# mrafidashti/neuradar

Hardware: NVIDIA B200
Metric: train_step_rays_per_sec (higher is better)
Workload: dtype f32

## Files before the change

neuradar_b200/csrc/field_fused.cu:

```cuda
#include <algorithm>
#include <cstdlib>

#include <cuda.h>
#include <cuda_bf16.h>

#include "actor_grid.cuh"
#include "hash_bwd_plan.cuh"
#include "tc_common.cuh"

namespace nrb {

using namespace tc;

struct FusedParams {
  const float* w[5];
  const float* b[5];
  const float* beta;
  float beta_min;
};

__device__ constexpr int kLK[5] = {32, 32, 48, 32, 32};
__device__ constexpr int kLN[5] = {32, 48, 32, 32, 32};
__device__ constexpr int kLOut[5] = {32, 33, 32, 32, 32};

// ... 145 lines not shown
    int agid = -1;
    if constexpr (kActors) agid = __ldg(a.as.grid_id + rr);
    if (kActors && agid >= 0) {
      float o16[16];
      actor_gather16(a.ag, agid, __ldg(a.as.pos + 3 * rr), __ldg(a.as.pos + 3 * rr + 1), __ldg(a.as.pos + 3 * rr + 2),
                     __ldg(a.as.std + rr), o16);
#pragma unroll
      for (int j = 0; j < 16; ++j) {
        v[j] = o16[j];
        v[16 + j] = 0.0f;
      }
    } else if constexpr (F > 0) {
      const float px = __ldg(a.xyz + 3 * rr), py = __ldg(a.xyz + 3 * rr + 1), pz = __ldg(a.xyz + 3 * rr + 2);
      const float sd = a.std != nullptr ? __ldg(a.std + rr) : 0.0f;
      const uint32_t hmask = (1u << grid.log2_size) - 1u;
      constexpr int kBatch = 8 / F;
#pragma unroll
      for (int l0 = 0; l0 < 32 / F; l0 += kBatch) {
        Cell c[kBatch];
        float f[kBatch][8][F];
#pragma unroll
        for (int i = 0; i < kBatch; ++i) {
          c[i] = locate_cell(px, py, pz, grid.scalings[l0 + i], hmask);
          const float* base = grid.table + (static_cast<size_t>(l0 + i) << grid.log2_size) * F;
#pragma unroll
          for (int k = 0; k < 8; ++k) load_row<F>(base, c[i].row[k], f[i][k]);
        }
#pragma unroll
        for (int i = 0; i < kBatch; ++i) {
          const float ax = c[i].ox, bx = 1.0f - c[i].ox, ay = c[i].oy, by = 1.0f - c[i].oy, az = c[i].oz, bz = 1.0f - c[i].oz;
          const float w = a.std != nullptr ? level_weight(grid.scalings[l0 + i], sd) : 1.0f;
#pragma unroll
          for (int j = 0; j < F; ++j) {
            const float f03 = f[i][0][j] * ax + f[i][3][j] * bx;
            const float f12 = f[i][1][j] * ax + f[i][2][j] * bx;
            const float f56 = f[i][5][j] * ax + f[i][6][j] * bx;
            const float f47 = f[i][4][j] * ax + f[i][7][j] * bx;
            const float f0312 = f03 * ay + f12 * by;
            const float f4756 = f47 * ay + f56 * by;
            v[(l0 + i) * F + j] = (f0312 * az + f4756 * bz) * w;
          }
        }
      }
    } else {
      float4 pf[8];
      warp_load_rows_coalesced(a.x, tile * kRows + (uwarp & 3) * 32, a.M, lane, pf);
      warp_bounce_to_rows(bounce, lane, pf, v);
    }
    tmem_store_row_split<32>(tg, uwarp, kFAHi, kFALo, 0, v);
    if (train) {
#pragma unroll
      for (int q = 0; q < 4; ++q) {
        uint32_t h[4], m[4];
#pragma unroll
        for (int c = 0; c < 4; ++c) split_bf16_pair(v[8 * q + 2 * c], v[8 * q + 2 * c + 1], h[c], m[c]);
        uint4* dst = a.ximg + tile * 1024 + q * 128 + r;
        dst[0] = make_uint4(h[0], h[1], h[2], h[3]);
        dst[512] = make_uint4(m[0], m[1], m[2], m[3]);
      }
    }
    auto relu_mask = [&](const float* bias) {
      uint32_t m = 0;
#pragma unroll
      for (int j = 0; j < 32; ++j) {
        v[j] = fmaxf(v[j] + bias[j], 0.0f);
        m |= (v[j] > 0.0f ? 1u : 0u) << j;
      }
      return m;
    };
    run_layer(0);
    tmem_load_row<32>(tg + kFAcc, uwarp, 0, v);
    const uint32_t m_h1 = relu_mask(s_bias);
    tmem_store_row_split<32>(tg, uwarp, kFAHi, kFALo, 0, v);
    run_layer(1);
    float sdf_v;
    float emb[32];
    {
      float geo[48];
      tmem_load_row<48>(tg + kFAcc, uwarp, 0, geo);
      sdf_v = geo[0] + s_bias[48];
#pragma unroll
      for (int j = 0; j < 32; ++j) emb[j] = geo[1 + j] + s_bias[48 + 1 + j];
    }
    tmem_store_row_split<32>(tg, uwarp, kFAHi, kFALo, 0, emb);
    {
      float shv[16];
      if (kActors && agid >= 0) {
        sh16_of_direction(__ldg(a.as.dirs + 3 * rr), __ldg(a.as.dirs + 3 * rr + 1), __ldg(a.as.dirs + 3 * rr + 2), shv);
      } else {
        const float4* shp = reinterpret_cast<const float4*>(a.sh + (rr / a.samples_per_ray) * 16);
#pragma unroll
        for (int c = 0; c < 4; ++c) {
          const float4 q4 = __ldg(shp + c);
          shv[4 * c] = q4.x;
          shv[4 * c + 1] = q4.y;
          shv[4 * c + 2] = q4.z;
          shv[4 * c + 3] = q4.w;
        }
      }
      tmem_store_row_split<16>(tg, uwarp, kFAHi, kFALo, 32, shv);
    }
    run_layer(2);
    tmem_load_row<32>(tg + kFAcc, uwarp, 0, v);
    const uint32_t m_g1 = relu_mask(s_bias + 2 * 48);
    tmem_store_row_split<32>(tg, uwarp, kFAHi, kFALo, 0, v);
    run_layer(3);
    tmem_load_row<32>(tg + kFAcc, uwarp, 0, v);
    const uint32_t m_g2 = relu_mask(s_bias + 3 * 48);
    tmem_store_row_split<32>(tg, uwarp, kFAHi, kFALo, 0, v);
    if (train && ok) {
      a.masks[row] = m_h1;
      a.masks[a.ld + row] = m_g1;
      a.masks[2 * a.ld + row] = m_g2;
    }
    run_layer(4);
    tmem_load_row<32>(tg + kFAcc, uwarp, 0, v);
#pragma unroll
    for (int j = 0; j < 32; ++j) v[j] = emb[j] + (v[j] + s_bias[4 * 48 + j]);
    warp_store_rows_coalesced(a.feature, tile * kRows + (uwarp & 3) * 32, a.M, bounce, lane, v);
    if (ok) {
      a.sdf[row] = sdf_v;
      a.alpha[row] = 1.0f / (1.0f + expf(sdf_v * beta));
    }
  }
  fence_before_sync();
  __syncthreads();
  if (uwarp == 0) tmem_free<512>(*tmem_slot);
}

constexpr int kBGroups = 2;
constexpr int kBWorkers = kBGroups * kRows;
constexpr int kBIssuers = 1;
constexpr int kBThreads = kBWorkers + kBIssuers * 32;
constexpr int kBCols = 112;
constexpr int kBAcc = 0, kBAHi = 32, kBAMid = 56, kBDHi = 80, kBDMid = 96;
__device__ constexpr int kDwCol[5] = {224, 224, 368, 296, 296};
__device__ constexpr int kDwLane[5] = {0, 16, 0, 0, 16};
constexpr int kSdfCol = 368, kSdfLane = 16;

struct FusedBwdSmem {
  static constexpr int d_hi = 0, d_mid = 8192;
  static constexpr int d_sdf = 16384;
  static constexpr int d_bytes = 18432;
  static constexpr int h1 = d_bytes;
  static constexpr int emb = h1 + 18432;
  static constexpr int g1 = emb + 26624;
  static constexpr int g2x = g1 + 18432;
  static constexpr int group_bytes = g2x + 18432;
  static constexpr int w = kBGroups * group_bytes;
  static constexpr int w_bytes = 4 * 4096 + 6144;
  static constexpr int w1row0 = w + w_bytes;
  static constexpr int bias = w1row0 + 128;
  static constexpr int mbar = bias + 5 * 48 * 4;
  static constexpr int tmem = mbar + 8 * 26;
  static constexpr int total = tmem + 16;
};
__host__ __device__ constexpr int fb_w_off(int l) { return l <= 2 ? l * 4096 : 4096 * 2 + 6144 + (l - 3) * 4096; }
__host__ __device__ constexpr int fb_w_half(int l) { return l == 2 ? 3072 : 2048; }
__device__ constexpr int kSlotOff[5] = {FusedBwdSmem::g2x, FusedBwdSmem::h1, FusedBwdSmem::emb, FusedBwdSmem::g1,
                                        FusedBwdSmem::g2x};
__device__ constexpr int kSlotMid[5] = {10240, 10240, 14336, 10240, 10240};

struct FusedBwdArgs {
  const uint4* ximg;
  const uint32_t* masks;
  int64_t ld;
  const float* sh;
  const float* sdf;
  const float* alpha;
  const float* dfeature;
  const float* dfeat_ray;
  const float* weights;
  const float* dsdf;
  const float* dalpha;
  int samples_per_ray;
  int64_t M;
  const int32_t* actor_grid_id;
  const float* actor_dirs;
  float4* dximg;
  float* dw[5];
  float* db[5];
  float* dbeta;
};

__device__ __forceinline__ void tmem_st16(uint32_t taddr, const uint32_t (&v)[16]) {
  asm volatile(
      "tcgen05.st.sync.aligned.32x32b.x16.b32 [%0], {%1, %2, %3, %4, %5, %6, %7, %8, %9, %10, %11, %12, %13, %14, %15, %16};" ::"r"(taddr),
      "r"(v[0]), "r"(v[1]), "r"(v[2]), "r"(v[3]), "r"(v[4]), "r"(v[5]), "r"(v[6]), "r"(v[7]), "r"(v[8]), "r"(v[9]), "r"(v[10]),
      "r"(v[11]), "r"(v[12]), "r"(v[13]), "r"(v[14]), "r"(v[15])
      : "memory");
}

__device__ __forceinline__ void tma_load_rows(void* dst_smem, const CUtensorMap* map, int32_t row0, uint64_t* mbar) {
  asm volatile(
      "cp.async.bulk.tensor.2d.shared::cluster.global.tile.mbarrier::complete_tx::bytes [%0], [%1, {%2, %3}], [%4];" ::"r"(
          smem_u32(dst_smem)),
      "l"(map), "r"(0), "r"(row0), "r"(smem_u32(mbar))
      : "memory");
}

#ifdef NRB_FUSED_TRACE
__device__ long long g_fused_trace[4096];
#define NRB_FT(slot)                                                                                            \
  do {                                                                                                          \
    if (blockIdx.x == 0 && t == 0 && trace_n < 2000) g_fused_trace[trace_n++] = (static_cast<long long>(slot) << 48) | (clock64() & 0xFFFFFFFFFFFFll); \
  } while (0)
#define NRB_FTI(slot)                                                                                           \
  do {                                                                                                          \
    if (blockIdx.x == 0 && uwarp == 8 && itrace_n < 4000) g_fused_trace[itrace_n++] = (static_cast<long long>(slot) << 48) | (clock64() & 0xFFFFFFFFFFFFll); \
  } while (0)
#else
#define NRB_FT(slot)
#define NRB_FTI(slot)
#endif

__global__ void __maxnreg__(128) field_fused_bwd_kernel(const __grid_constant__ FusedParams prm,
                                                                       const __grid_constant__ FusedBwdArgs a,
                                                                       const __grid_constant__ CUtensorMap dfeat_map) {
  extern __shared__ __align__(1024) char smem[];
  const int t = threadIdx.x, lane = t & 31, r = t & (kRows - 1);
  const int uwarp = uniform_warp_idx();
#ifdef NRB_FUSED_TRACE
  int trace_n = 0, itrace_n = 2000;
#endif
  uint64_t* mbars = reinterpret_cast<uint64_t*>(smem + FusedBwdSmem::mbar);
  uint64_t* mb_data = mbars;
  uint64_t* mb_xfull = mbars + 2;
  uint64_t* mb_dfull = mbars + 4;
  uint64_t* mb_ready = mbars + 6;
  uint64_t* mb_done = mbars + 16;
  uint32_t* tmem_slot = reinterpret_cast<uint32_t*>(smem + FusedBwdSmem::tmem);
  float* s_bias = reinterpret_cast<float*>(smem + FusedBwdSmem::bias);
  float* w1row0 = reinterpret_cast<float*>(smem + FusedBwdSmem::w1row0);

  for (int l = 0; l < 5; ++l) {
    const int K = kLK[l];
    const float* src = prm.w[l] + (l == 1 ? 32 : 0);
    char* hi = smem + FusedBwdSmem::w + fb_w_off(l);
    char* mid = hi + fb_w_half(l);
    for (int e = t; e < 32 * K / 2; e += kBThreads) {
      const int n = e / (K / 2), k = 2 * (e - n * (K / 2));
      uint32_t h, m;
      split_bf16_pair(__ldg(src + n * K + k), __ldg(src + n * K + k + 1), h, m);
      const int off = (n >> 3) * (K / 8) * 128 + (k >> 3) * 128 + (n & 7) * 16 + (k & 7) * 2;
      *reinterpret_cast<uint32_t*>(hi + off) = h;
      *reinterpret_cast<uint32_t*>(mid + off) = m;
    }
    for (int j = t; j < 48; j += kBThreads) s_bias[l * 48 + j] = (j < kLOut[l] && prm.b[l] != nullptr) ? __ldg(prm.b[l] + j) : 0.0f;
  }
  if (t < 32) w1row0[t] = __ldg(prm.w[1] + t);
  for (int gq = 0; gq < kBGroups; ++gq) {
    char* base = smem + gq * FusedBwdSmem::group_bytes;
    for (int e = t; e < 4 * 128; e += kBThreads) {
      const int slot = e >> 7, s = e & 127;
      const int off = slot == 0 ? FusedBwdSmem::h1 + 8192 : slot == 1 ? FusedBwdSmem::emb + 12288
                      : slot == 2 ? FusedBwdSmem::g1 + 8192 : FusedBwdSmem::g2x + 8192;
      *reinterpret_cast<uint4*>(base + off + s * 16) = make_uint4(0x00003F80u, 0u, 0u, 0u);
    }
  }
  if (uwarp == 0) tmem_alloc<512>(tmem_slot);
  if (t == 0) {
    for (int i = 0; i < 6; ++i) mbar_init(mbars + i, 1);
    for (int i = 0; i < 10; ++i) mbar_init(mb_ready + i, kRows);
    for (int i = 0; i < 10; ++i) mbar_init(mb_done + i, 1);
  }
  fence_async_smem();
  fence_before_sync();
  __syncthreads();
  fence_after_sync();
  const uint32_t tmem_base = *tmem_slot;
  const int64_t tiles = (a.M + kRows - 1) / kRows;
  const int64_t mine = static_cast<int64_t>(blockIdx.x) < tiles ? (tiles - 1 - blockIdx.x) / gridDim.x + 1 : 0;

  if (uwarp >= 8) {
    const int64_t cnt[2] = {(mine + 1) / 2, mine / 2};
    int64_t it[2] = {0, 0};
    int lcur[2] = {4, 4};
    bool pend[2] = {false, false};
    uint32_t used = 0;
    while (it[0] < cnt[0] || it[1] < cnt[1] || pend[0] || pend[1]) {
      bool progressed = false;
#pragma unroll
      for (int gq = 0; gq < 2; ++gq) {
        char* gsq = smem + gq * FusedBwdSmem::group_bytes;
        if (pend[gq] && mbar_test(mb_done + gq * 5 + 4, static_cast<uint32_t>(it[gq] & 1))) {
          if (elect_one()) {
            const int64_t tile = blockIdx.x + (2 * it[gq] + gq) * gridDim.x;
            mbar_expect_tx(mb_xfull + gq, 16384);
            bulk_load(gsq + FusedBwdSmem::g2x, a.ximg + tile * 1024, 8192, mb_xfull + gq);
            bulk_load(gsq + FusedBwdSmem::g2x + 10240, a.ximg + tile * 1024 + 512, 8192, mb_xfull + gq);
          }
          __syncwarp();
          pend[gq] = false;
          progressed = true;
        }
        if (it[gq] < cnt[gq] && mbar_test(mb_ready + gq * 5 + lcur[gq], static_cast<uint32_t>(it[gq] & 1))) {
          const int l = lcur[gq];
          if (elect_one()) {
            NRB_FTI(100 + gq);
            fence_after_sync();
            const uint32_t base = smem_u32(gsq);
            const uint32_t d_tmem = tmem_base + (static_cast<uint32_t>(kDwLane[l]) << 16) + static_cast<uint32_t>(kDwCol[l]);
            const uint32_t idesc = idesc_bf16(64, 2 * kLK[l] + 8, 1, 1);
            uint64_t da = make_desc(base + FusedBwdSmem::d_hi, 128, 2048), db = make_desc(base + kSlotOff[l], 128, 2048);
            const bool acc0 = (used >> l) & 1u;
#pragma unroll
            for (int ks = 0; ks < kRows / 16; ++ks) {
              mma_bf16_ss(d_tmem, da, db, idesc, acc0 || ks > 0);
              da += 16;
              db += 16;
            }
            if (l == 1) {
              const uint32_t s_tmem = tmem_base + (static_cast<uint32_t>(kSdfLane) << 16) + static_cast<uint32_t>(kSdfCol);
              uint64_t sa = make_desc(base + FusedBwdSmem::d_sdf, 128, 2048), sb = make_desc(base + kSlotOff[1], 128, 2048);
#pragma unroll
              for (int ks = 0; ks < kRows / 16; ++ks) {
                mma_bf16_ss(s_tmem, sa, sb, idesc, acc0 || ks > 0);
                sa += 16;
                sb += 16;
              }
            }
            mma_commit(mb_done + gq * 5 + l);
            NRB_FTI(110 + gq);
          }
          __syncwarp();
          used |= 1u << l;
          if (l == 4) pend[gq] = true;
          if (l == 0) {
            lcur[gq] = 4;
            ++it[gq];
          } else {
            lcur[gq] = l - 1;
          }
          progressed = true;
        }
      }
      if (!progressed) __nanosleep(64);
    }
  } else {
    const int g = uwarp >> 2, wq = uwarp & 3;
    char* gs = smem + g * FusedBwdSmem::group_bytes;
    const uint32_t tg = tmem_base + static_cast<uint32_t>(g * kBCols);
    const uint32_t lane_base = tg + (static_cast<uint32_t>(wq * 32) << 16);
    const float beta = fabsf(__ldg(prm.beta)) + prm.beta_min;
    const bool rank1 = a.dfeature == nullptr;
    uint32_t ph_data = 0;
    float dbeta_acc = 0.0f;

    auto data_step = [&](auto&& issue) {
      fence_before_sync();
      group_barrier(g);
      if (wq == 0) {
        if (elect_one()) {
          fence_after_sync();
          issue();
          mma_commit(mb_data + g);
        }
        __syncwarp();
      }
      mbar_wait(mb_data + g, ph_data);
      ph_data ^= 1;
      fence_after_sync();
    };
    auto issue_fwd = [&](int l) {
      const int K = kLK[l];
      const uint32_t idesc = idesc_bf16(128, 32, 0, 0);
      const uint32_t wb = smem_u32(smem + FusedBwdSmem::w + fb_w_off(l));
      uint64_t bh = make_desc(wb, 128, (K / 8) * 128), bm = make_desc(wb + fb_w_half(l), 128, (K / 8) * 128);
      for (int ks = 0; ks < K / 16; ++ks) {
        mma_bf16_ts(tg + kBAcc, tg + kBAMid + 8 * ks, bh, idesc, ks > 0);
        mma_bf16_ts(tg + kBAcc, tg + kBAHi + 8 * ks, bm, idesc, true);
        mma_bf16_ts(tg + kBAcc, tg + kBAHi + 8 * ks, bh, idesc, true);
        bh += 16;
        bm += 16;
      }
    };
    auto issue_din = [&](int l) {
      const int K = kLK[l];
      const uint32_t idesc = idesc_bf16(128, 32, 0, 1);
      const uint32_t wb = smem_u32(smem + FusedBwdSmem::w + fb_w_off(l));
      const uint32_t kgroup = static_cast<uint32_t>((K / 8) * 128);
      uint64_t bh = make_desc(wb, kgroup, 128), bm = make_desc(wb + fb_w_half(l), kgroup, 128);
      for (int ks = 0; ks < 2; ++ks) {
        mma_bf16_ts(tg + kBAcc, tg + kBDMid + 8 * ks, bh, idesc, ks > 0);
        mma_bf16_ts(tg + kBAcc, tg + kBDHi + 8 * ks, bm, idesc, true);
        mma_bf16_ts(tg + kBAcc, tg + kBDHi + 8 * ks, bh, idesc, true);
        bh += (2 * kgroup) >> 4;
        bm += (2 * kgroup) >> 4;
      }
    };
    auto stage_row32 = [&](const float (&v)[32], int col_hi, int col_mid, char* img_hi, char* img_mid) {
      uint32_t h[16], m[16];
#pragma unroll
      for (int c = 0; c < 16; ++c) split_bf16_pair(v[2 * c], v[2 * c + 1], h[c], m[c]);
      if (col_hi >= 0) {
        tmem_st16(lane_base + static_cast<uint32_t>(col_hi), h);
        tmem_st16(lane_base + static_cast<uint32_t>(col_mid), m);
      }
#pragma unroll
      for (int q = 0; q < 4; ++q) {
        *reinterpret_cast<uint4*>(img_hi + q * 2048 + r * 16) = make_uint4(h[4 * q], h[4 * q + 1], h[4 * q + 2], h[4 * q + 3]);
        *reinterpret_cast<uint4*>(img_mid + q * 2048 + r * 16) = make_uint4(m[4 * q], m[4 * q + 1], m[4 * q + 2], m[4 * q + 3]);
      }
      if (col_hi >= 0) tmem_st_wait();
    };
    auto load_acc = [&](float (&v)[32]) { tmem_load_row<32>(tg + kBAcc, uwarp, 0, v); };
    auto wait_done = [&](int l, int64_t it) { mbar_wait(mb_done + g * 5 + l, static_cast<uint32_t>(it & 1)); };
    auto signal_ready = [&](int l) {
      fence_async_smem();
      mbar_arrive(mb_ready + g * 5 + l);
    };

    uint4 xq[8];
    uint32_t m_h1 = 0, m_g1 = 0, m_g2 = 0;
    auto load_head = [&](int64_t tile) {
      const int64_t rc = min(tile * kRows + r, a.M - 1);
      const uint4* src = a.ximg + tile * 1024 + r;
#pragma unroll
      for (int q = 0; q < 4; ++q) {
        xq[q] = __ldg(src + q * 128);
        xq[4 + q] = __ldg(src + 512 + q * 128);
      }
      m_h1 = __ldg(a.masks + rc), m_g1 = __ldg(a.masks + a.ld + rc), m_g2 = __ldg(a.masks + 2 * a.ld + rc);
    };
    if (g < mine) load_head(blockIdx.x + static_cast<int64_t>(g) * gridDim.x);

    int64_t it = 0;
    for (int64_t k = g; k < mine; k += 2, ++it) {
      const int64_t tile = blockIdx.x + k * gridDim.x;
      const int64_t row = tile * kRows + r;
      const bool ok = row < a.M;
      const int64_t rc = ok ? row : (a.M - 1);
      float v[32];
      NRB_FT(0);
      if (it > 0) wait_done(0, it - 1);
      if (!rank1 && r == 0) {
        mbar_expect_tx(mb_dfull + g, 16384);
        tma_load_rows(gs + FusedBwdSmem::d_hi, &dfeat_map, static_cast<int32_t>(tile * kRows), mb_dfull + g);
      }
      {
        const uint32_t ha[16] = {xq[0].x, xq[0].y, xq[0].z, xq[0].w, xq[1].x, xq[1].y, xq[1].z, xq[1].w,
                                 xq[2].x, xq[2].y, xq[2].z, xq[2].w, xq[3].x, xq[3].y, xq[3].z, xq[3].w};
        const uint32_t ma[16] = {xq[4].x, xq[4].y, xq[4].z, xq[4].w, xq[5].x, xq[5].y, xq[5].z, xq[5].w,
                                 xq[6].x, xq[6].y, xq[6].z, xq[6].w, xq[7].x, xq[7].y, xq[7].z, xq[7].w};
        tmem_st16(lane_base + kBAHi, ha);
        tmem_st16(lane_base + kBAMid, ma);
        tmem_st_wait();
      }
      const uint32_t mh1 = m_h1, mg1 = m_g1, mg2 = m_g2;
      float4 shq[4];
      if (a.actor_grid_id != nullptr && __ldg(a.actor_grid_id + rc) >= 0) {
        float o[16];
        sh16_of_direction(__ldg(a.actor_dirs + 3 * rc), __ldg(a.actor_dirs + 3 * rc + 1), __ldg(a.actor_dirs + 3 * rc + 2), o);
#pragma unroll
        for (int c = 0; c < 4; ++c) shq[c] = make_float4(o[4 * c], o[4 * c + 1], o[4 * c + 2], o[4 * c + 3]);
      } else {
        const float4* shp = reinterpret_cast<const float4*>(a.sh + (rc / a.samples_per_ray) * 16);
#pragma unroll
        for (int c = 0; c < 4; ++c) shq[c] = __ldg(shp + c);
      }
      NRB_FT(10);
      data_step([&] { issue_fwd(0); });
      NRB_FT(20);
      load_acc(v);
#pragma unroll
      for (int j = 0; j < 32; ++j) v[j] = ((mh1 >> j) & 1u) ? v[j] + s_bias[j] : 0.0f;
      stage_row32(v, kBAHi, kBAMid, gs + FusedBwdSmem::h1, gs + FusedBwdSmem::h1 + 10240);
      NRB_FT(11);
      data_step([&] { issue_fwd(1); });
      NRB_FT(21);
      load_acc(v);
#pragma unroll
      for (int j = 0; j < 32; ++j) v[j] += s_bias[48 + 1 + j];
      stage_row32(v, kBAHi, kBAMid, gs + FusedBwdSmem::emb, gs + FusedBwdSmem::emb + 14336);
      {
        uint32_t h[8], m[8];
#pragma unroll
        for (int c = 0; c < 4; ++c) {
          split_bf16_pair(shq[c].x, shq[c].y, h[2 * c], m[2 * c]);
          split_bf16_pair(shq[c].z, shq[c].w, h[2 * c + 1], m[2 * c + 1]);
        }
#pragma unroll
        for (int q = 0; q < 2; ++q) {
          const uint32_t hq[4] = {h[4 * q], h[4 * q + 1], h[4 * q + 2], h[4 * q + 3]};
          const uint32_t mq[4] = {m[4 * q], m[4 * q + 1], m[4 * q + 2], m[4 * q + 3]};
          tmem_st4(lane_base + static_cast<uint32_t>(kBAHi + 16 + 4 * q), hq);
          tmem_st4(lane_base + static_cast<uint32_t>(kBAMid + 16 + 4 * q), mq);
          *reinterpret_cast<uint4*>(gs + FusedBwdSmem::emb + (4 + q) * 2048 + r * 16) = make_uint4(hq[0], hq[1], hq[2], hq[3]);
          *reinterpret_cast<uint4*>(gs + FusedBwdSmem::emb + 14336 + (4 + q) * 2048 + r * 16) = make_uint4(mq[0], mq[1], mq[2], mq[3]);
        }
        tmem_st_wait();
      }
      NRB_FT(12);
      data_step([&] { issue_fwd(2); });
      NRB_FT(22);
      load_acc(v);
#pragma unroll
      for (int j = 0; j < 32; ++j) v[j] = ((mg1 >> j) & 1u) ? v[j] + s_bias[2 * 48 + j] : 0.0f;
      stage_row32(v, kBAHi, kBAMid, gs + FusedBwdSmem::g1, gs + FusedBwdSmem::g1 + 10240);
      NRB_FT(13);
      data_step([&] { issue_fwd(3); });
      NRB_FT(23);
      load_acc(v);
#pragma unroll
      for (int j = 0; j < 32; ++j) v[j] = ((mg2 >> j) & 1u) ? v[j] + s_bias[3 * 48 + j] : 0.0f;
      stage_row32(v, -1, -1, gs + FusedBwdSmem::g2x, gs + FusedBwdSmem::g2x + 10240);

      float demb[32];
      NRB_FT(50);
      if (!rank1) {
        mbar_wait(mb_dfull + g, static_cast<uint32_t>(it & 1));
        const char* rowp = gs + FusedBwdSmem::d_hi + r * 128;
#pragma unroll
        for (int c = 0; c < 8; ++c) {
          const float4 q4 = *reinterpret_cast<const float4*>(rowp + ((c ^ (r & 7)) << 4));
          demb[4 * c] = q4.x;
          demb[4 * c + 1] = q4.y;
          demb[4 * c + 2] = q4.z;
          demb[4 * c + 3] = q4.w;
        }
        group_barrier(g);
      } else {
        const float wgt = __ldg(a.weights + rc);
        const float4* dfp = reinterpret_cast<const float4*>(a.dfeat_ray + (rc / a.samples_per_ray) * 32);
#pragma unroll
        for (int c = 0; c < 8; ++c) {
          const float4 q4 = __ldg(dfp + c);
          demb[4 * c] = wgt * q4.x;
          demb[4 * c + 1] = wgt * q4.y;
          demb[4 * c + 2] = wgt * q4.z;
          demb[4 * c + 3] = wgt * q4.w;
        }
      }
#pragma unroll
      for (int j = 0; j < 32; ++j) demb[j] = ok ? demb[j] : 0.0f;
      stage_row32(demb, kBDHi, kBDMid, gs + FusedBwdSmem::d_hi, gs + FusedBwdSmem::d_mid);
      signal_ready(4);
      float a_v = 0.0f, sd_v = 0.0f, da_v = 0.0f, ds_v = 0.0f;
      if (ok) {
        a_v = __ldg(a.alpha + row), sd_v = __ldg(a.sdf + row);
        da_v = a.dalpha != nullptr ? __ldg(a.dalpha + row) : 0.0f;
        ds_v = a.dsdf != nullptr ? __ldg(a.dsdf + row) : 0.0f;
      }
      NRB_FT(34);
      data_step([&] { issue_din(4); });
      NRB_FT(44);
      load_acc(v);
#pragma unroll
      for (int j = 0; j < 32; ++j) v[j] = ((mg2 >> j) & 1u) ? v[j] : 0.0f;
      NRB_FT(54);
      wait_done(4, it);
      NRB_FT(64);
      stage_row32(v, kBDHi, kBDMid, gs + FusedBwdSmem::d_hi, gs + FusedBwdSmem::d_mid);
      signal_ready(3);
      NRB_FT(33);
      data_step([&] { issue_din(3); });
      NRB_FT(43);
      load_acc(v);
#pragma unroll
      for (int j = 0; j < 32; ++j) v[j] = ((mg1 >> j) & 1u) ? v[j] : 0.0f;
      NRB_FT(53);
      wait_done(3, it);
      NRB_FT(63);
      stage_row32(v, kBDHi, kBDMid, gs + FusedBwdSmem::d_hi, gs + FusedBwdSmem::d_mid);
      signal_ready(2);
      NRB_FT(32);
      data_step([&] { issue_din(2); });
      NRB_FT(42);
      load_acc(v);
#pragma unroll
      for (int j = 0; j < 32; ++j) demb[j] += v[j];
      float dsdf_v = 0.0f;
      if (ok) {
        const float sg = a_v * (1.0f - a_v);
        dsdf_v = ds_v - da_v * beta * sg;
        dbeta_acc -= da_v * sd_v * sg;
      }
      NRB_FT(52);
      wait_done(2, it);
      NRB_FT(62);
      stage_row32(demb, kBDHi, kBDMid, gs + FusedBwdSmem::d_hi, gs + FusedBwdSmem::d_mid);
      {
        uint32_t h, m;
        split_bf16_pair(dsdf_v, 0.0f, h, m);
        *reinterpret_cast<uint4*>(gs + FusedBwdSmem::d_sdf + r * 16) = make_uint4((h & 0xFFFFu) | (m << 16), 0u, 0u, 0u);
      }
      signal_ready(1);
      NRB_FT(31);
      data_step([&] { issue_din(1); });
      NRB_FT(41);
      load_acc(v);
#pragma unroll
      for (int j = 0; j < 32; ++j) {
        const float d = fmaf(dsdf_v, w1row0[j], v[j]);
        v[j] = ((mh1 >> j) & 1u) ? d : 0.0f;
      }
      NRB_FT(51);
      wait_done(1, it);
      NRB_FT(61);
      stage_row32(v, kBDHi, kBDMid, gs + FusedBwdSmem::d_hi, gs + FusedBwdSmem::d_mid);
      NRB_FT(70);
      mbar_wait(mb_xfull + g, static_cast<uint32_t>(it & 1));
      NRB_FT(71);
      signal_ready(0);
      if (k + 2 < mine) load_head(blockIdx.x + (k + 2) * gridDim.x);
      if (a.dximg != nullptr) {
        NRB_FT(30);
        data_step([&] { issue_din(0); });
        NRB_FT(40);
        load_acc(v);
        float4* dst = a.dximg + tile * 1024 + r;
#pragma unroll
        for (int c = 0; c < 8; ++c) dst[c * 128] = make_float4(v[4 * c], v[4 * c + 1], v[4 * c + 2], v[4 * c + 3]);
      }
    }
    if (it > 0) wait_done(0, it - 1);
    const float sb = warp_sum(dbeta_acc);
    if (lane == 0 && a.dbeta != nullptr && sb != 0.0f) {
      const float b0 = __ldg(prm.beta);
      atomicAdd(a.dbeta, sb * (b0 > 0.0f ? 1.0f : (b0 < 0.0f ? -1.0f : 0.0f)));
    }
  }
  fence_before_sync();
  __syncthreads();
  fence_after_sync();
  if (mine > 0 && uwarp < 4) {
    const int wq = uwarp, half = lane >> 4, j = wq * 16 + (lane & 15);
#pragma unroll
    for (int u = 0; u < 6; ++u) {
      const int l = u < 5 ? u : 1;
      const int K = u < 5 ? kLK[u] : 32;
      const int col = u < 5 ? kDwCol[u] : kSdfCol, lane_off = u < 5 ? kDwLane[u] : kSdfLane;
      const uint32_t taddr = tmem_base + (static_cast<uint32_t>(wq * 32) << 16) + static_cast<uint32_t>(col);
      const int wrow = u == 5 ? 0 : (u == 1 ? (j & 31) + 1 : (j & 31));
      const bool mine_row = (half == (lane_off >> 4)) && (u == 5 ? j < 2 : true);
#pragma unroll
      for (int c = 0; c < 6; ++c) {
        if (c * 8 < K) {
          float hi8[8], mid8[8];
          tmem_ld8(taddr + c * 8, hi8);
          tmem_ld8(taddr + K + 8 + c * 8, mid8);
          tmem_ld_wait();
          if (mine_row && a.dw[l] != nullptr) {
#pragma unroll
            for (int i = 0; i < 8; ++i) atomicAdd(a.dw[l] + wrow * K + c * 8 + i, hi8[i] + mid8[i]);
          }
        }
      }
      float b8[8];
      tmem_ld8(taddr + K, b8);
      tmem_ld_wait();
      if (mine_row && a.db[l] != nullptr) atomicAdd(a.db[l] + wrow, b8[0]);
    }
  }
  fence_before_sync();
  __syncthreads();
  if (uwarp == 0) tmem_free<512>(tmem_base);
}

}

using namespace nrb;

static FusedParams fused_params(const nrb_field_mlp_t* p) {
  FusedParams prm;
  for (int l = 0; l < 5; ++l) {
    prm.w[l] = p->weights[l];
    prm.b[l] = p->biases[l];
  }
  prm.beta = p->beta;
  prm.beta_min = p->beta_min;
  return prm;
}


static int make_rows_tensor_map(CUtensorMap* map, const float* base, int64_t M) {
  using EncodeFn = CUresult (*)(CUtensorMap*, CUtensorMapDataType, cuuint32_t, void*, const cuuint64_t*, const cuuint64_t*,
                                const cuuint32_t*, const cuuint32_t*, CUtensorMapInterleave, CUtensorMapSwizzle,
                                CUtensorMapL2promotion, CUtensorMapFloatOOBfill);
  static EncodeFn encode = nullptr;
  if (encode == nullptr) {
    void* fn = nullptr;
    cudaDriverEntryPointQueryResult qres;
    cudaError_t e = cudaGetDriverEntryPoint("cuTensorMapEncodeTiled", &fn, cudaEnableDefault, &qres);
    NRB_REQUIRE(e == cudaSuccess && fn != nullptr, NRB_ERR_UNSUPPORTED, "cuTensorMapEncodeTiled is not available: %s",
                cudaGetErrorString(e));
    encode = reinterpret_cast<EncodeFn>(fn);
  }
  const cuuint64_t dims[2] = {32, static_cast<cuuint64_t>(M)};
  const cuuint64_t strides[1] = {128};
  const cuuint32_t box[2] = {32, 128};
  const cuuint32_t estr[2] = {1, 1};
  const CUresult r = encode(map, CU_TENSOR_MAP_DATA_TYPE_FLOAT32, 2, const_cast<float*>(base), dims, strides, box, estr,
                            CU_TENSOR_MAP_INTERLEAVE_NONE, CU_TENSOR_MAP_SWIZZLE_128B, CU_TENSOR_MAP_L2_PROMOTION_L2_128B,
                            CU_TENSOR_MAP_FLOAT_OOB_FILL_NONE);
  NRB_REQUIRE(r == CUDA_SUCCESS, NRB_ERR_BAD_ARG, "cuTensorMapEncodeTiled failed with CUresult %d", static_cast<int>(r));
  return NRB_OK;
}

extern "C" int64_t nrb_field_saved_ld(int64_t M) { return (M + tc::kRows - 1) / tc::kRows * tc::kRows; }

extern "C" int64_t nrb_field_fused_image_bytes(int64_t M) { return (M + tc::kRows - 1) / tc::kRows * 16384; }

extern "C" int nrb_field_fused_fwd(const nrb_field_mlp_t* p, const nrb_grid_t* grid, const float* xyz, const float* std,
                                   const float* x, const float* sh, int32_t samples_per_ray, int64_t M, float* feature,
                                   float* sdf, float* alpha, const nrb_field_fused_saved_t* saved,
                                   const nrb_actor_grids_t* actor_grids, const nrb_actor_samples_t* actor_samples,
                                   nrb_stream_t stream) {
  NRB_REQUIRE(p && sh && feature && sdf && alpha && M >= 0 && samples_per_ray > 0, NRB_ERR_BAD_ARG,
              "nrb_field_fused_fwd: null pointer or bad size");
  for (int l = 0; l < 5; ++l) NRB_REQUIRE(p->weights[l] != nullptr, NRB_ERR_BAD_ARG, "nrb_field_fused_fwd: weights[%d] is null", l);
  NRB_REQUIRE(p->beta != nullptr, NRB_ERR_BAD_ARG, "nrb_field_fused_fwd: beta is null");
  NRB_REQUIRE((grid != nullptr) != (x != nullptr), NRB_ERR_BAD_ARG,
              "nrb_field_fused_fwd: pass either a grid (+ xyz) to gather from or the hash features x");
  int F = 0;
  GridDev gd{};
  if (grid != nullptr) {
    if (int rc = check_grid(grid)) return rc;
    NRB_REQUIRE(xyz != nullptr, NRB_ERR_BAD_ARG, "nrb_field_fused_fwd: xyz is null");
    F = grid->features_per_level;
    NRB_REQUIRE((F == 2 || F == 4) && grid->num_levels * F == 32, NRB_ERR_UNSUPPORTED,
                "nrb_field_fused_fwd: the fused gather needs num_levels * features_per_level == 32 with 2 or 4 features");
    gd = to_dev(grid);
  } else {
    NRB_REQUIRE(aligned16(x), NRB_ERR_ALIGNMENT, "nrb_field_fused_fwd: x must be 16-byte aligned");
  }
  NRB_REQUIRE(aligned16(sh) && aligned16(feature), NRB_ERR_ALIGNMENT, "nrb_field_fused_fwd: sh and feature must be 16-byte aligned");
  if (M == 0) return NRB_OK;
  FusedFwdArgs a{};
  a.xyz = xyz, a.std = std, a.x = x, a.sh = sh, a.samples_per_ray = samples_per_ray, a.M = M;
  a.feature = feature, a.sdf = sdf, a.alpha = alpha;
  if (saved != nullptr && saved->ximg != nullptr) {
    NRB_REQUIRE(saved->masks != nullptr && saved->ld >= M && saved->ld % tc::kRows == 0 && aligned16(saved->ximg),
                NRB_ERR_BAD_ARG, "nrb_field_fused_fwd: saved.masks / saved.ld (nrb_field_saved_ld(M)) / alignment");
    a.ximg = static_cast<uint4*>(saved->ximg), a.masks = saved->masks, a.ld = saved->ld;
  }
  const bool actors = actor_grids != nullptr;
  if (actors) {
    if (int rc = check_actor_grids("nrb_field_fused_fwd", actor_grids)) return rc;
    NRB_REQUIRE(grid != nullptr && actor_samples && actor_samples->grid_id && actor_samples->pos && actor_samples->std &&
                    actor_samples->dirs,
                NRB_ERR_BAD_ARG, "nrb_field_fused_fwd: actors need the gather mode and all per-sample actor arrays");
    a.ag = to_dev(actor_grids);
    a.as = ActorSamplesDev{actor_samples->grid_id, actor_samples->pos, actor_samples->std, actor_samples->dirs};
  }
  const int64_t tiles = (M + tc::kRows - 1) / tc::kRows;
  const unsigned nblk = static_cast<unsigned>(std::min<int64_t>((tiles + kFGroups - 1) / kFGroups, sm_count()));
  auto s = static_cast<cudaStream_t>(stream);
#define NRB_FUSED_FWD(FF, AA)                                                                                                  \
  {                                                                                                                            \
    cudaError_t e = ensure_dynamic_smem(reinterpret_cast<const void*>(field_fused_fwd_kernel<FF, AA>), FusedFwdSmem::total); \
    NRB_REQUIRE(e == cudaSuccess, static_cast<int>(e), "nrb_field_fused_fwd: cudaFuncSetAttribute: %s", cudaGetErrorString(e));  \
    field_fused_fwd_kernel<FF, AA><<<nblk, kFThreads, FusedFwdSmem::total, s>>>(fused_params(p), gd, a);                       \
  }
  if (F == 2 && actors) NRB_FUSED_FWD(2, true) else if (F == 4 && actors) NRB_FUSED_FWD(4, true)
  else if (F == 2) NRB_FUSED_FWD(2, false) else if (F == 4) NRB_FUSED_FWD(4, false) else NRB_FUSED_FWD(0, false)
#undef NRB_FUSED_FWD
  return finish_launch("nrb_field_fused_fwd");
// ... 51 lines not shown
```

neuradar_b200/csrc/tc_common.cuh:

```cuda
#pragma once

#include "common.cuh"

namespace nrb {
namespace tc {

constexpr int kRows = 128;

__device__ __forceinline__ uint32_t smem_u32(const void* p) {
  return static_cast<uint32_t>(__cvta_generic_to_shared(p));
}

__device__ __forceinline__ uint64_t make_desc(uint32_t saddr, uint32_t lbo_bytes, uint32_t sbo_bytes) {
  uint64_t d = 0;
  d |= static_cast<uint64_t>((saddr & 0x3FFFFu) >> 4);
  d |= static_cast<uint64_t>((lbo_bytes >> 4) & 0x3FFFu) << 16;
  d |= static_cast<uint64_t>((sbo_bytes >> 4) & 0x3FFFu) << 32;
  d |= static_cast<uint64_t>(1) << 46;
  return d;
}

__device__ __forceinline__ uint32_t make_idesc(int n, int a_mn_major, int b_mn_major) {
  return (1u << 4) | (2u << 7) | (2u << 10) | (static_cast<uint32_t>(a_mn_major) << 15) |
         (static_cast<uint32_t>(b_mn_major) << 16) | (static_cast<uint32_t>(n >> 3) << 17) | ((128u >> 4) << 24);
// ... 335 lines not shown
      const float send = upper ? v[i] : v[i + s];
      const float keep = upper ? v[i + s] : v[i];
      v[i] = keep + __shfl_xor_sync(kFull, send, s);
    }
  }
  return v[0];
}


__device__ __forceinline__ void tmem_ld8(uint32_t taddr, float (&v)[8]) {
  uint32_t r[8];
  asm volatile("tcgen05.ld.sync.aligned.32x32b.x8.b32 {%0, %1, %2, %3, %4, %5, %6, %7}, [%8];"
               : "=r"(r[0]), "=r"(r[1]), "=r"(r[2]), "=r"(r[3]), "=r"(r[4]), "=r"(r[5]), "=r"(r[6]), "=r"(r[7])
               : "r"(taddr));
#pragma unroll
  for (int i = 0; i < 8; ++i) v[i] = __uint_as_float(r[i]);
}

template <int W>
__device__ __forceinline__ void tmem_load_cols(uint32_t tmem_base, int warp, int col0, float (&v)[W]) {
  const uint32_t taddr = tmem_base + (static_cast<uint32_t>((warp & 3) * 32) << 16) + static_cast<uint32_t>(col0);
  if constexpr (W == 8) {
    tmem_ld8(taddr, v);
  } else {
#pragma unroll
    for (int c = 0; c < W / 16; ++c) {
      float t[16];
      tmem_ld16(taddr + c * 16, t);
#pragma unroll
      for (int i = 0; i < 16; ++i) v[c * 16 + i] = t[i];
    }
  }
  tmem_ld_wait();
}

template <int W>
__device__ __forceinline__ void store_row_part_split(char* hi_tile, char* lo_tile, int row, int K, int col0,
                                                     const float (&v)[W]) {
#pragma unroll
  for (int c = 0; c < W / 4; ++c) {
    const float4 h = make_float4(tf32_hi(v[4 * c]), tf32_hi(v[4 * c + 1]), tf32_hi(v[4 * c + 2]), tf32_hi(v[4 * c + 3]));
    const float4 l = make_float4(v[4 * c] - h.x, v[4 * c + 1] - h.y, v[4 * c + 2] - h.z, v[4 * c + 3] - h.w);
    const uint32_t off = tile_offset(row, (col0 >> 2) + c, K);
    *reinterpret_cast<float4*>(hi_tile + off) = h;
    *reinterpret_cast<float4*>(lo_tile + off) = l;
  }
}

template <int W>
__device__ __forceinline__ void store_part_transposed_split(char* hi_tile, char* lo_tile, int quarter, int lane,
                                                            const float (&v)[W], int row_offset) {
  const int i = lane & 3;
  const int c4 = quarter * 8 + (lane >> 2);
#pragma unroll
  for (int g = 0; g < W / 4; ++g) {
    float a0 = v[4 * g], a1 = v[4 * g + 1], a2 = v[4 * g + 2], a3 = v[4 * g + 3];
    {
      const bool odd = (i & 1) != 0;
      const float s01 = odd ? a0 : a1, s23 = odd ? a2 : a3;
      const float r01 = __shfl_xor_sync(kFull, s01, 1), r23 = __shfl_xor_sync(kFull, s23, 1);
      if (odd) {
        a0 = r01;
        a2 = r23;
      } else {
        a1 = r01;
        a3 = r23;
      }
    }
    {
      const bool up = (i & 2) != 0;
      const float s0 = up ? a0 : a2, s1 = up ? a1 : a3;
      const float r0 = __shfl_xor_sync(kFull, s0, 2), r1 = __shfl_xor_sync(kFull, s1, 2);
      if (up) {
        a0 = r0;
        a1 = r1;
      } else {
        a2 = r0;
        a3 = r1;
      }
    }
    const float4 h = make_float4(tf32_hi(a0), tf32_hi(a1), tf32_hi(a2), tf32_hi(a3));
    const float4 l = make_float4(a0 - h.x, a1 - h.y, a2 - h.z, a3 - h.w);
    const uint32_t off = tile_offset(row_offset + 4 * g + i, c4, kRows);
    *reinterpret_cast<float4*>(hi_tile + off) = h;
    *reinterpret_cast<float4*>(lo_tile + off) = l;
  }
}

template <int W>
__device__ __forceinline__ int bounce_swizzle(int row) {
  constexpr int CPR = W / 4, RP = 8 / CPR;
  return (row / RP) % CPR;
}

template <int W>
__device__ __forceinline__ void warp_load_part_coalesced(const float* __restrict__ g, int64_t row_base, int64_t M, int col0,
                                                         int lane, float4 (&pf)[W / 4]) {
  constexpr int CPR = W / 4, RPI = 32 / CPR;
#pragma unroll
  for (int q = 0; q < CPR; ++q) {
    const int64_t r = min(row_base + q * RPI + lane / CPR, M - 1);
    pf[q] = __ldg(reinterpret_cast<const float4*>(g + r * 32 + col0) + (lane % CPR));
  }
}

template <int W>
__device__ __forceinline__ void warp_bounce_part_to_rows(char* bounce, int lane, const float4 (&pf)[W / 4], float (&v)[W]) {
  constexpr int CPR = W / 4, RPI = 32 / CPR;
#pragma unroll
  for (int q = 0; q < CPR; ++q) {
    const int r = q * RPI + lane / CPR, cc = lane % CPR;
    *reinterpret_cast<float4*>(bounce + r * (W * 4) + ((cc ^ bounce_swizzle<W>(r)) << 4)) = pf[q];
  }
  __syncwarp();
#pragma unroll
  for (int cc = 0; cc < CPR; ++cc) {
    const float4 t = *reinterpret_cast<const float4*>(bounce + lane * (W * 4) + ((cc ^ bounce_swizzle<W>(lane)) << 4));
    v[4 * cc] = t.x;
    v[4 * cc + 1] = t.y;
    v[4 * cc + 2] = t.z;
    v[4 * cc + 3] = t.w;
  }
  __syncwarp();
}

template <int W>
__device__ __forceinline__ void warp_store_part_coalesced(float* __restrict__ g, int64_t row_base, int64_t M, int col0,
                                                          char* bounce, int lane, const float (&v)[W]) {
  constexpr int CPR = W / 4, RPI = 32 / CPR;
#pragma unroll
  for (int cc = 0; cc < CPR; ++cc)
    *reinterpret_cast<float4*>(bounce + lane * (W * 4) + ((cc ^ bounce_swizzle<W>(lane)) << 4)) =
        make_float4(v[4 * cc], v[4 * cc + 1], v[4 * cc + 2], v[4 * cc + 3]);
  __syncwarp();
#pragma unroll
  for (int q = 0; q < CPR; ++q) {
    const int r = q * RPI + lane / CPR, cc = lane % CPR;
    const float4 t = *reinterpret_cast<const float4*>(bounce + r * (W * 4) + ((cc ^ bounce_swizzle<W>(r)) << 4));
    if (row_base + r < M) reinterpret_cast<float4*>(g + (row_base + r) * 32 + col0)[cc] = t;
  }
  __syncwarp();
}


__device__ __forceinline__ void tmem_st8(uint32_t taddr, const float (&v)[8]) {
  asm volatile("tcgen05.st.sync.aligned.32x32b.x8.b32 [%0], {%1, %2, %3, %4, %5, %6, %7, %8};" ::"r"(taddr),
               "r"(__float_as_uint(v[0])), "r"(__float_as_uint(v[1])), "r"(__float_as_uint(v[2])),
               "r"(__float_as_uint(v[3])), "r"(__float_as_uint(v[4])), "r"(__float_as_uint(v[5])),
               "r"(__float_as_uint(v[6])), "r"(__float_as_uint(v[7]))
               : "memory");
}
__device__ __forceinline__ void tmem_st_wait() { asm volatile("tcgen05.wait::st.sync.aligned;" ::: "memory"); }

template <int W>
__device__ __forceinline__ void tmem_store_row_split(uint32_t tmem_base, int warp, int hi_col, int lo_col, int col,
                                                     const float (&v)[W]) {
  const uint32_t lane_base = tmem_base + (static_cast<uint32_t>((warp & 3) * 32) << 16);
#pragma unroll
  for (int c = 0; c < W / 8; ++c) {
    float hi[8], lo[8];
#pragma unroll
    for (int i = 0; i < 8; ++i) {
      hi[i] = tf32_hi(v[8 * c + i]);
      lo[i] = v[8 * c + i] - hi[i];
    }
    tmem_st8(lane_base + static_cast<uint32_t>(hi_col + col + 8 * c), hi);
    tmem_st8(lane_base + static_cast<uint32_t>(lo_col + col + 8 * c), lo);
  }
  tmem_st_wait();
}

__device__ __forceinline__ void mma_tf32_ts(uint32_t d_tmem, uint32_t a_tmem, uint64_t b_desc, uint32_t idesc,
                                            bool accumulate) {
  asm volatile(
      "{\n\t"
      ".reg .pred p;\n\t"
      "setp.ne.b32 p, %4, 0;\n\t"
      "tcgen05.mma.cta_group::1.kind::tf32 [%0], [%1], %2, %3, p;\n\t"
      "}\n" ::"r"(d_tmem),
      "r"(a_tmem), "l"(b_desc), "r"(idesc), "r"(static_cast<uint32_t>(accumulate))
      : "memory");
}

__device__ __forceinline__ void issue_gemm_ts(uint32_t d_tmem, int n, uint32_t a_hi_tmem, uint32_t a_lo_tmem, uint32_t b_hi,
                                              uint32_t b_lo, int b_cols, int k_red) {
  const uint32_t idesc = make_idesc_m(128, n, 0, 0);
  const uint32_t b_sbo = static_cast<uint32_t>(b_cols / 4) * 128u;
  uint64_t bh = make_desc(b_hi, 128, b_sbo), bl = make_desc(b_lo, 128, b_sbo);
  bool acc = false;
#pragma unroll 4
  for (int k = 0; k < k_red / 8; ++k) {
    mma_tf32_ts(d_tmem, a_lo_tmem + 8 * k, bh, idesc, acc);
    mma_tf32_ts(d_tmem, a_hi_tmem + 8 * k, bl, idesc, true);
    mma_tf32_ts(d_tmem, a_hi_tmem + 8 * k, bh, idesc, true);
    acc = true;
    bh += 16;
    bl += 16;
  }
}

}
}
```

Baseline: 15.64 million.

## Bulk-load input image into smem and tcgen05.cp to TMEM; cut register cap to 96

Replaces the per-thread register prefetch of the input image (8 uint4 per thread) with a bulk async copy into shared memory tracked by a new mbarrier, followed by tcgen05.cp into TMEM issued inside the MMA data step. The demb gradient is parked in TMEM instead of registers across the backward layers, and stage_row32 is split into halves to shorten live ranges. It also narrows loop counters to int and defers the beta load. Together these allow the register cap to drop from 128 to 96, aimed at reducing register pressure and spills. The risk is extra TMEM traffic and new barrier waits, and the smem slot reuse (g1) must not race with other stages.

```diff
diff --git a/neuradar_b200/csrc/field_fused.cu b/neuradar_b200/csrc/field_fused.cu
--- a/neuradar_b200/csrc/field_fused.cu
+++ b/neuradar_b200/csrc/field_fused.cu
@@ -321,7 +321,7 @@
   static constexpr int w1row0 = w + w_bytes;
   static constexpr int bias = w1row0 + 128;
   static constexpr int mbar = bias + 5 * 48 * 4;
-  static constexpr int tmem = mbar + 8 * 26;
+  static constexpr int tmem = mbar + 8 * 28;
   static constexpr int total = tmem + 16;
 };
 __host__ __device__ constexpr int fb_w_off(int l) { return l <= 2 ? l * 4096 : 4096 * 2 + 6144 + (l - 3) * 4096; }
@@ -352,6 +352,12 @@
   float* dbeta;
 };
 
+__device__ __forceinline__ void tmem_st8(uint32_t taddr, const uint32_t (&v)[8]) {
+  asm volatile("tcgen05.st.sync.aligned.32x32b.x8.b32 [%0], {%1, %2, %3, %4, %5, %6, %7, %8};" ::"r"(taddr), "r"(v[0]),
+               "r"(v[1]), "r"(v[2]), "r"(v[3]), "r"(v[4]), "r"(v[5]), "r"(v[6]), "r"(v[7])
+               : "memory");
+}
+
 __device__ __forceinline__ void tmem_st16(uint32_t taddr, const uint32_t (&v)[16]) {
   asm volatile(
       "tcgen05.st.sync.aligned.32x32b.x16.b32 [%0], {%1, %2, %3, %4, %5, %6, %7, %8, %9, %10, %11, %12, %13, %14, %15, %16};" ::"r"(taddr),
@@ -383,7 +389,7 @@
 #define NRB_FTI(slot)
 #endif
 
-__global__ void __maxnreg__(128) field_fused_bwd_kernel(const __grid_constant__ FusedParams prm,
+__global__ void __maxnreg__(96) field_fused_bwd_kernel(const __grid_constant__ FusedParams prm,
                                                                        const __grid_constant__ FusedBwdArgs a,
                                                                        const __grid_constant__ CUtensorMap dfeat_map) {
   extern __shared__ __align__(1024) char smem[];
@@ -398,6 +404,7 @@
   uint64_t* mb_dfull = mbars + 4;
   uint64_t* mb_ready = mbars + 6;
   uint64_t* mb_done = mbars + 16;
+  uint64_t* mb_head = mbars + 26;
   uint32_t* tmem_slot = reinterpret_cast<uint32_t*>(smem + FusedBwdSmem::tmem);
   float* s_bias = reinterpret_cast<float*>(smem + FusedBwdSmem::bias);
   float* w1row0 = reinterpret_cast<float*>(smem + FusedBwdSmem::w1row0);
@@ -432,6 +439,7 @@
     for (int i = 0; i < 6; ++i) mbar_init(mbars + i, 1);
     for (int i = 0; i < 10; ++i) mbar_init(mb_ready + i, kRows);
     for (int i = 0; i < 10; ++i) mbar_init(mb_done + i, 1);
+    for (int i = 0; i < 2; ++i) mbar_init(mb_head + i, 1);
   }
   fence_async_smem();
   fence_before_sync();
@@ -439,7 +447,7 @@
   fence_after_sync();
   const uint32_t tmem_base = *tmem_slot;
   const int64_t tiles = (a.M + kRows - 1) / kRows;
-  const int64_t mine = static_cast<int64_t>(blockIdx.x) < tiles ? (tiles - 1 - blockIdx.x) / gridDim.x + 1 : 0;
+  const int mine = static_cast<int64_t>(blockIdx.x) < tiles ? static_cast<int>((tiles - 1 - blockIdx.x) / gridDim.x + 1) : 0;
 
   if (uwarp >= 8) {
     const int64_t cnt[2] = {(mine + 1) / 2, mine / 2};
@@ -511,7 +519,6 @@
     char* gs = smem + g * FusedBwdSmem::group_bytes;
     const uint32_t tg = tmem_base + static_cast<uint32_t>(g * kBCols);
     const uint32_t lane_base = tg + (static_cast<uint32_t>(wq * 32) << 16);
-    const float beta = fabsf(__ldg(prm.beta)) + prm.beta_min;
     const bool rank1 = a.dfeature == nullptr;
     uint32_t ph_data = 0;
     float dbeta_acc = 0.0f;
@@ -559,44 +566,51 @@
       }
     };
     auto stage_row32 = [&](const float (&v)[32], int col_hi, int col_mid, char* img_hi, char* img_mid) {
-      uint32_t h[16], m[16];
-#pragma unroll
-      for (int c = 0; c < 16; ++c) split_bf16_pair(v[2 * c], v[2 * c + 1], h[c], m[c]);
-      if (col_hi >= 0) {
-        tmem_st16(lane_base + static_cast<uint32_t>(col_hi), h);
-        tmem_st16(lane_base + static_cast<uint32_t>(col_mid), m);
-      }
-#pragma unroll
-      for (int q = 0; q < 4; ++q) {
-        *reinterpret_cast<uint4*>(img_hi + q * 2048 + r * 16) = make_uint4(h[4 * q], h[4 * q + 1], h[4 * q + 2], h[4 * q + 3]);
-        *reinterpret_cast<uint4*>(img_mid + q * 2048 + r * 16) = make_uint4(m[4 * q], m[4 * q + 1], m[4 * q + 2], m[4 * q + 3]);
+#pragma unroll
+      for (int half = 0; half < 2; ++half) {
+        uint32_t h[8], m[8];
+#pragma unroll
+        for (int c = 0; c < 8; ++c) split_bf16_pair(v[16 * half + 2 * c], v[16 * half + 2 * c + 1], h[c], m[c]);
+        if (col_hi >= 0) {
+          tmem_st8(lane_base + static_cast<uint32_t>(col_hi + 8 * half), h);
+          tmem_st8(lane_base + static_cast<uint32_t>(col_mid + 8 * half), m);
+        }
+#pragma unroll
+        for (int q = 0; q < 2; ++q) {
+          const int o = (2 * half + q) * 2048 + r * 16;
+          *reinterpret_cast<uint4*>(img_hi + o) = make_uint4(h[4 * q], h[4 * q + 1], h[4 * q + 2], h[4 * q + 3]);
+          *reinterpret_cast<uint4*>(img_mid + o) = make_uint4(m[4 * q], m[4 * q + 1], m[4 * q + 2], m[4 * q + 3]);
+        }
       }
       if (col_hi >= 0) tmem_st_wait();
     };
     auto load_acc = [&](float (&v)[32]) { tmem_load_row<32>(tg + kBAcc, uwarp, 0, v); };
-    auto wait_done = [&](int l, int64_t it) { mbar_wait(mb_done + g * 5 + l, static_cast<uint32_t>(it & 1)); };
+    auto wait_done = [&](int l, int it) { mbar_wait(mb_done + g * 5 + l, static_cast<uint32_t>(it & 1)); };
     auto signal_ready = [&](int l) {
       fence_async_smem();
       mbar_arrive(mb_ready + g * 5 + l);
     };
 
-    uint4 xq[8];
     uint32_t m_h1 = 0, m_g1 = 0, m_g2 = 0;
-    auto load_head = [&](int64_t tile) {
+    auto fetch_image = [&](int64_t tile) {
+      if (r == 0) {
+        mbar_expect_tx(mb_head + g, 16384);
+        bulk_load(gs + FusedBwdSmem::g1, a.ximg + tile * 1024, 8192, mb_head + g);
+        bulk_load(gs + FusedBwdSmem::g1 + 10240, a.ximg + tile * 1024 + 512, 8192, mb_head + g);
+      }
+    };
+    auto load_masks = [&](int64_t tile) {
       const int64_t rc = min(tile * kRows + r, a.M - 1);
-      const uint4* src = a.ximg + tile * 1024 + r;
-#pragma unroll
-      for (int q = 0; q < 4; ++q) {
-        xq[q] = __ldg(src + q * 128);
-        xq[4 + q] = __ldg(src + 512 + q * 128);
-      }
       m_h1 = __ldg(a.masks + rc), m_g1 = __ldg(a.masks + a.ld + rc), m_g2 = __ldg(a.masks + 2 * a.ld + rc);
     };
-    if (g < mine) load_head(blockIdx.x + static_cast<int64_t>(g) * gridDim.x);
-
-    int64_t it = 0;
-    for (int64_t k = g; k < mine; k += 2, ++it) {
-      const int64_t tile = blockIdx.x + k * gridDim.x;
+    if (g < mine) {
+      fetch_image(blockIdx.x + static_cast<int64_t>(g) * gridDim.x);
+      load_masks(blockIdx.x + static_cast<int64_t>(g) * gridDim.x);
+    }
+
+    int it = 0;
+    for (int k = g; k < mine; k += 2, ++it) {
+      const int64_t tile = blockIdx.x + static_cast<int64_t>(k) * gridDim.x;
       const int64_t row = tile * kRows + r;
       const bool ok = row < a.M;
       const int64_t rc = ok ? row : (a.M - 1);
@@ -607,15 +621,6 @@
         mbar_expect_tx(mb_dfull + g, 16384);
         tma_load_rows(gs + FusedBwdSmem::d_hi, &dfeat_map, static_cast<int32_t>(tile * kRows), mb_dfull + g);
       }
-      {
-        const uint32_t ha[16] = {xq[0].x, xq[0].y, xq[0].z, xq[0].w, xq[1].x, xq[1].y, xq[1].z, xq[1].w,
-                                 xq[2].x, xq[2].y, xq[2].z, xq[2].w, xq[3].x, xq[3].y, xq[3].z, xq[3].w};
-        const uint32_t ma[16] = {xq[4].x, xq[4].y, xq[4].z, xq[4].w, xq[5].x, xq[5].y, xq[5].z, xq[5].w,
-                                 xq[6].x, xq[6].y, xq[6].z, xq[6].w, xq[7].x, xq[7].y, xq[7].z, xq[7].w};
-        tmem_st16(lane_base + kBAHi, ha);
-        tmem_st16(lane_base + kBAMid, ma);
-        tmem_st_wait();
-      }
       const uint32_t mh1 = m_h1, mg1 = m_g1, mg2 = m_g2;
       float4 shq[4];
       if (a.actor_grid_id != nullptr && __ldg(a.actor_grid_id + rc) >= 0) {
@@ -629,19 +634,17 @@
         for (int c = 0; c < 4; ++c) shq[c] = __ldg(shp + c);
       }
       NRB_FT(10);
-      data_step([&] { issue_fwd(0); });
+      data_step([&] {
+        mbar_wait(mb_head + g, static_cast<uint32_t>(it & 1));
+        const uint32_t xs = smem_u32(gs + FusedBwdSmem::g1);
+#pragma unroll
+        for (int h = 0; h < 2; ++h) {
+          tmem_cp_128x256b(tg + kBAHi + 8 * h, make_desc(xs + h * 4096, 2048, 128));
+          tmem_cp_128x256b(tg + kBAMid + 8 * h, make_desc(xs + 10240 + h * 4096, 2048, 128));
+        }
+        issue_fwd(0);
+      });
       NRB_FT(20);
-      load_acc(v);
-#pragma unroll
-      for (int j = 0; j < 32; ++j) v[j] = ((mh1 >> j) & 1u) ? v[j] + s_bias[j] : 0.0f;
-      stage_row32(v, kBAHi, kBAMid, gs + FusedBwdSmem::h1, gs + FusedBwdSmem::h1 + 10240);
-      NRB_FT(11);
-      data_step([&] { issue_fwd(1); });
-      NRB_FT(21);
-      load_acc(v);
-#pragma unroll
-      for (int j = 0; j < 32; ++j) v[j] += s_bias[48 + 1 + j];
-      stage_row32(v, kBAHi, kBAMid, gs + FusedBwdSmem::emb, gs + FusedBwdSmem::emb + 14336);
       {
         uint32_t h[8], m[8];
 #pragma unroll
@@ -658,8 +661,18 @@
           *reinterpret_cast<uint4*>(gs + FusedBwdSmem::emb + (4 + q) * 2048 + r * 16) = make_uint4(hq[0], hq[1], hq[2], hq[3]);
           *reinterpret_cast<uint4*>(gs + FusedBwdSmem::emb + 14336 + (4 + q) * 2048 + r * 16) = make_uint4(mq[0], mq[1], mq[2], mq[3]);
         }
-        tmem_st_wait();
-      }
+      }
+      load_acc(v);
+#pragma unroll
+      for (int j = 0; j < 32; ++j) v[j] = ((mh1 >> j) & 1u) ? v[j] + s_bias[j] : 0.0f;
+      stage_row32(v, kBAHi, kBAMid, gs + FusedBwdSmem::h1, gs + FusedBwdSmem::h1 + 10240);
+      NRB_FT(11);
+      data_step([&] { issue_fwd(1); });
+      NRB_FT(21);
+      load_acc(v);
+#pragma unroll
+      for (int j = 0; j < 32; ++j) v[j] += s_bias[48 + 1 + j];
+      stage_row32(v, kBAHi, kBAMid, gs + FusedBwdSmem::emb, gs + FusedBwdSmem::emb + 14336);
       NRB_FT(12);
       data_step([&] { issue_fwd(2); });
       NRB_FT(22);
@@ -703,10 +716,20 @@
       }
 #pragma unroll
       for (int j = 0; j < 32; ++j) demb[j] = ok ? demb[j] : 0.0f;
+      {
+        uint32_t p[16];
+#pragma unroll
+        for (int h = 0; h < 2; ++h) {
+#pragma unroll
+          for (int j = 0; j < 16; ++j) p[j] = __float_as_uint(demb[16 * h + j]);
+          tmem_st16(lane_base + static_cast<uint32_t>(kBAHi + 16 * h), p);
+        }
+      }
       stage_row32(demb, kBDHi, kBDMid, gs + FusedBwdSmem::d_hi, gs + FusedBwdSmem::d_mid);
       signal_ready(4);
-      float a_v = 0.0f, sd_v = 0.0f, da_v = 0.0f, ds_v = 0.0f;
+      float a_v = 0.0f, sd_v = 0.0f, da_v = 0.0f, ds_v = 0.0f, beta = 0.0f;
       if (ok) {
+        beta = fabsf(__ldg(prm.beta)) + prm.beta_min;
         a_v = __ldg(a.alpha + row), sd_v = __ldg(a.sdf + row);
         da_v = a.dalpha != nullptr ? __ldg(a.dalpha + row) : 0.0f;
         ds_v = a.dsdf != nullptr ? __ldg(a.dsdf + row) : 0.0f;
@@ -731,12 +754,14 @@
       NRB_FT(53);
       wait_done(3, it);
       NRB_FT(63);
+      if (k + 2 < mine) fetch_image(tile + 2 * gridDim.x);
       stage_row32(v, kBDHi, kBDMid, gs + FusedBwdSmem::d_hi, gs + FusedBwdSmem::d_mid);
       signal_ready(2);
       NRB_FT(32);
       data_step([&] { issue_din(2); });
       NRB_FT(42);
       load_acc(v);
+      tmem_load_row<32>(tg + kBAHi, uwarp, 0, demb);
 #pragma unroll
       for (int j = 0; j < 32; ++j) demb[j] += v[j];
       float dsdf_v = 0.0f;
@@ -772,7 +797,7 @@
       mbar_wait(mb_xfull + g, static_cast<uint32_t>(it & 1));
       NRB_FT(71);
       signal_ready(0);
-      if (k + 2 < mine) load_head(blockIdx.x + (k + 2) * gridDim.x);
+      if (k + 2 < mine) load_masks(tile + 2 * gridDim.x);
       if (a.dximg != nullptr) {
         NRB_FT(30);
         data_step([&] { issue_din(0); });
diff --git a/neuradar_b200/csrc/tc_common.cuh b/neuradar_b200/csrc/tc_common.cuh
--- a/neuradar_b200/csrc/tc_common.cuh
+++ b/neuradar_b200/csrc/tc_common.cuh
@@ -511,6 +511,10 @@
 }
 __device__ __forceinline__ void tmem_st_wait() { asm volatile("tcgen05.wait::st.sync.aligned;" ::: "memory"); }
 
+__device__ __forceinline__ void tmem_cp_128x256b(uint32_t taddr, uint64_t s_desc) {
+  asm volatile("tcgen05.cp.cta_group::1.128x256b [%0], %1;" ::"r"(taddr), "l"(s_desc) : "memory");
+}
+
 template <int W>
 __device__ __forceinline__ void tmem_store_row_split(uint32_t tmem_base, int warp, int hi_col, int lo_col, int col,
                                                      const float (&v)[W]) {
```

Result: faster. 15.92 million, median of 6 (+1.8%).
